# ChenDavidTimothy/mujoco-template

Hardware: AMD Instinct MI355X
Metric: env-steps/sec (whole node), humanoid batch=4096 random-ctrl rollout (higher is better)
Workload: dtype f32

## Files before the change

mujoco_template_amd/csrc/mjb_device.hpp:

```cpp
#pragma once
#include "mjb_types.hpp"

#ifdef MJB_HOST_EMU
#include <cmath>
#include "mjb_hostemu.hpp"
#define MJB_DEV static inline
#define MJB_DEVM inline
#define MJB_DEV_CALL static __attribute__((noinline))
#else
#include <hip/hip_runtime.h>
#define MJB_DEV __device__ __forceinline__
#define MJB_DEVM __device__ __forceinline__
#define MJB_DEV_CALL __device__ __attribute__((noinline))
#endif

#ifdef MJB_HOST_EMU
#define MJB_MFMA(a, b, acc) emu_mfma((a), (b), (acc))
#define MJB_BALLOT(p) emu_ballot(p)
#define MJB_RSQF(x) (1.0f / sqrtf(x))
#define MJB_RCPF(x) (1.0f / (x))
#define MJB_MEMTIME() 0ull
#define MJB_OPAQUE1(a) ((void)0)
#define MJB_OPAQUE2(a, b) ((void)0)
#define MJB_OPAQUE9(a, b, c, d, e, f, g, h, i) ((void)0)
// ... 1418 lines not shown
        if (t_abs(det) >= (sizeof(T) == 4 ? (T)1e-6 * ma * mc : Num<T>::minval())) {
          x1 = (mc * u - mb * v) / det; x2 = (ma * v - mb * u) / det;
          if (x1 > s1[1]) { x1 = s1[1]; x2 = (v - mb * s1[1]) / mc; }
          else if (x1 < -s1[1]) { x1 = -s1[1]; x2 = (v + mb * s1[1]) / mc; }
          if (x2 > s2[1]) { x2 = s2[1]; x1 = t_min(t_max((u - mb * s2[1]) / ma, -s1[1]), s1[1]); }
          else if (x2 < -s2[1]) { x2 = -s2[1]; x1 = t_min(t_max((u + mb * s2[1]) / ma, -s1[1]), s1[1]); }
          T v1[3] = {p1[0] + z1[0] * x1, p1[1] + z1[1] * x1, p1[2] + z1[2] * x1};
          T v2[3] = {p2[0] + z2[0] * x2, p2[1] + z2[1] * x2, p2[2] + z2[2] * x2};
          n = nc_sphere_sphere(v1, s1[0], v2, s2[0], margin, rc[0]);
        } else {
#pragma unroll
          for (int k = 0; k < 4; k++) {
            if (n >= 2) continue;
            bool ok;
            if (k < 2) { x1 = k == 0 ? s1[1] : -s1[1]; x2 = (v - mb * x1) / mc; ok = x2 >= -s2[1] && x2 <= s2[1]; }
            else { x2 = k == 2 ? s2[1] : -s2[1]; x1 = (u - mb * x2) / ma; ok = x1 >= -s1[1] && x1 <= s1[1]; }
            if (!ok) continue;
            T v1[3] = {p1[0] + z1[0] * x1, p1[1] + z1[1] * x1, p1[2] + z1[2] * x1};
            T v2[3] = {p2[0] + z2[0] * x2, p2[1] + z2[1] * x2, p2[2] + z2[2] * x2};
            RawCon<T> tmp;
            if (nc_sphere_sphere(v1, s1[0], v2, s2[0], margin, tmp)) { if (n == 0) rc[0] = tmp; else rc[1] = tmp; n++; }
          }
        }
      }
    }
    int total, off = gscan_small<G>(n, lane, total);
#pragma unroll
    for (int k = 0; k < 4; k++) {
      if (k < n) {
        int slot = ncon + off + k;
        if (slot < m.ncon_max) {
          const RawCon<T>& r = rc[k];
          T f[9] = {r.n[0], r.n[1], r.n[2], r.yh[0], r.yh[1], r.yh[2], 0, 0, 0};
          normalize3(f);
          if (dot3(f + 3, f + 3) < (T)0.25) {
            f[3] = f[4] = f[5] = 0;
            if (f[1] < (T)0.5 && f[1] > (T)-0.5) f[4] = 1; else f[5] = 1;
          }
          T d = dot3(f, f + 3);
          f[3] -= d * f[0]; f[4] -= d * f[1]; f[5] -= d * f[2];
          normalize3(f + 3);
          T* o = con + slot * CON_STRIDE;
          o[0] = r.dist; o[1] = r.pos[0]; o[2] = r.pos[1]; o[3] = r.pos[2];
#pragma unroll
          for (int a = 0; a < 6; a++) o[4 + a] = f[a];
          o[10] = prm_row<PRM_PAIR_FRICTION>(c, m.pair_friction, 5 * m.npair)[5 * p];
          con_pair[slot] = p;
        }
      }
    }
    int newn = ncon + total;
    if (newn > m.ncon_max) { dropped += newn - (ncon > m.ncon_max ? ncon : m.ncon_max); }
    ncon = newn;
  }
}

template <typename T, int G> MJB_DEV void collision(Ctx<T>& c) {
  MJB_ENV(c); T* w = c.w; const int lane = c.lane;
  T *gx = w + L.geom_xpos, *gm = w + L.geom_xmat;
  int ncon = 0, dropped = 0;
  if (m.nefc_max * m.nv < G) {
    for (int base = 0; base < m.npair; base += G) collide_pass<T, G>(c, base + lane, base + lane < m.npair, ncon, dropped);
  } else {
    int* cand = (int*)(w + L.efc_J);
    int nl = 0;
    for (int base = 0; base < m.npair; base += G) {
      const int p = base + lane;
      bool keep = false;
      if (p < m.npair) {
        const int g1 = m.pair_geom1[p], g2 = m.pair_geom2[p];
        const T cull = m.pair_cull[p];
        T d[3] = {gx[3 * g2] - gx[3 * g1], gx[3 * g2 + 1] - gx[3 * g1 + 1], gx[3 * g2 + 2] - gx[3 * g1 + 2]};
        if (cull < 0) {
          T nz[3] = {gm[9 * g1 + 2], gm[9 * g1 + 5], gm[9 * g1 + 8]};
          keep = dot3(d, nz) <= -cull * (T)1.00001 + (T)1e-6;
        } else {
          T r = cull * (T)1.00001 + (T)1e-6;
          keep = dot3(d, d) <= r * r;
        }
      }
      int total, off = gscan_small<G>(keep ? 1 : 0, lane, total);
      if (nl + total > G) {
        gsync<G>();
        collide_pass<T, G>(c, lane < nl ? cand[lane] : 0, lane < nl, ncon, dropped);
        gsync<G>();
        nl = 0;
      }
      if (keep) cand[nl + off] = p;
      nl += total;
    }
    gsync<G>();
    if (nl > 0) collide_pass<T, G>(c, lane < nl ? cand[lane] : 0, lane < nl, ncon, dropped);
  }
  c.con_dropped += dropped;
  c.ncon = ncon < m.ncon_max ? ncon : m.ncon_max;
  gsync<G>();
}

template <typename T> MJB_DEV void row_imp_R(T pos, T margin, const T* solimp, T diagApprox, T& imp, T& R) {
  T dmin = t_min(t_max(solimp[0], MJB_MINIMP), MJB_MAXIMP), dmax = t_min(t_max(solimp[1], MJB_MINIMP), MJB_MAXIMP);
  T width = t_max(solimp[2], (T)0), mid = t_min(t_max(solimp[3], MJB_MINIMP), MJB_MAXIMP), power = t_max(solimp[4], (T)1);
  if (dmin == dmax || width <= Num<T>::minval()) imp = (T)0.5 * (dmin + dmax);
  else {
    T x = t_abs(pos - margin) / width;
    if (x >= 1) imp = dmax;
    else if (x <= 0) imp = dmin;
    else {
      T y;
      if (power == 1) y = x;
#ifdef MJB_SPEC_SOLIMP_POWER_1_OR_2
      else y = x <= mid ? x * x / mid : 1 - (1 - x) * (1 - x) / (1 - mid);
#else
      else if (power == 2) y = x <= mid ? x * x / mid : 1 - (1 - x) * (1 - x) / (1 - mid);
      else if (x <= mid) y = t_pow(x, power) / t_pow(mid, power - 1);
      else y = 1 - t_pow(1 - x, power) / t_pow(1 - mid, power - 1);
#endif
      imp = dmin + y * (dmax - dmin);
    }
  }
  R = t_max(Num<T>::minval(), (1 - imp) * diagApprox / imp);
}
template <typename T> MJB_DEV void row_params(ModelRef<T> m, T pos, T margin, const T* solref, const T* solimp, T diagApprox, T& K, T& B, T& imp, T& R) {
  T dmin = t_min(t_max(solimp[0], MJB_MINIMP), MJB_MAXIMP), dmax = t_min(t_max(solimp[1], MJB_MINIMP), MJB_MAXIMP);
  T width = t_max(solimp[2], (T)0), mid = t_min(t_max(solimp[3], MJB_MINIMP), MJB_MAXIMP), power = t_max(solimp[4], (T)1);
  if (dmin == dmax || width <= Num<T>::minval()) imp = (T)0.5 * (dmin + dmax);
  else {
    T x = t_abs(pos - margin) / width;
    if (x >= 1) imp = dmax;
    else if (x <= 0) imp = dmin;
    else {
      T y;
      if (power == 1) y = x;
#ifdef MJB_SPEC_SOLIMP_POWER_1_OR_2
      else y = x <= mid ? x * x / mid : 1 - (1 - x) * (1 - x) / (1 - mid);
#else
      else if (power == 2) y = x <= mid ? x * x / mid : 1 - (1 - x) * (1 - x) / (1 - mid);
      else if (x <= mid) y = t_pow(x, power) / t_pow(mid, power - 1);
      else y = 1 - t_pow(1 - x, power) / t_pow(1 - mid, power - 1);
#endif
      imp = dmin + y * (dmax - dmin);
    }
  }
  if (solref[0] > 0) {
    T tc = t_max(solref[0], 2 * m.timestep), dr = solref[1];
    K = 1 / t_max(Num<T>::minval(), dmax * dmax * tc * tc * dr * dr);
    B = 2 / t_max(Num<T>::minval(), dmax * tc);
  } else {
    K = -solref[0] / t_max(Num<T>::minval(), dmax * dmax);
    B = -solref[1] / t_max(Num<T>::minval(), dmax);
  }
  R = t_max(Num<T>::minval(), (1 - imp) * diagApprox / imp);
}

template <typename T, int G> MJB_DEV void make_constraint(Ctx<T>& c) {
  MJB_ENV(c); T* w = c.w; const int lane = c.lane, nv = m.nv, cap = m.nefc_max;
  T *qpos = w + L.qpos, *qvel = w + L.qvel, *J = w + L.efc_J, *epos = w + L.efc_pos, *eD = w + L.efc_D, *earef = w + L.efc_aref;
  T *eK = w + L.efc_jar, *eB = w + L.efc_jv, *eI = w + L.efc_force;
  T *emargin = w + L.efc_KBI;
  int *etype = c.wi + L.i_efc_type, *con_pair = c.wi + L.i_con_pair;
  T *con = w + L.con, *tl = w + L.ten_length, *tj = w + L.ten_J;
  int nefc = 0, dropped = 0;
  {
    const int nobj = m.njnt + m.ntendon;
    for (int base = 0; base < nobj; base += G) {
      const int k = base + lane;
      const bool isj = k < m.njnt;
      const int o = isj ? k : k - m.njnt;
      int cnt = 0;
      T dist[2] = {0, 0}, margin = 0;
      bool act[2] = {false, false};
      T rec[12];
      if (k < nobj && m.lim_i[2 * k]) {
        const int vi = m.lim_i[2 * k + 1];
#pragma unroll
        for (int q = 0; q < 11; q++) rec[q] = m.lim_f[12 * k + q];
        T value = isj ? qpos[vi] : tl[vi];
        margin = rec[2];
        dist[0] = value - rec[0]; dist[1] = rec[1] - value;
        act[0] = dist[0] < margin; act[1] = dist[1] < margin;
        cnt = (int)act[0] + (int)act[1];
      }
      int total, off = gscan_small<G>(cnt, lane, total);
      int row = nefc + off;
      if (cnt > 0) {
#pragma unroll
        for (int sd = 0; sd < 2; sd++) {
          if (act[sd]) {
            if (row < cap) {
              T imp, R;
              row_imp_R(dist[sd], margin, rec + 6, rec[3], imp, R);
              etype[row] = (isj ? EFC_LIMIT_JOINT : EFC_LIMIT_TENDON) | ((o * 2 + sd) << 9);
              epos[row] = dist[sd]; emargin[row] = margin; eD[row] = 1 / R; eK[row] = rec[4]; eB[row] = rec[5]; eI[row] = imp;
            }
            row++;
          }
        }
      }
      int newn = nefc + total;
      if (newn > cap) dropped += newn - (nefc > cap ? nefc : cap);
      nefc = newn;
    }
  }
  if (nefc > cap) nefc = cap;
  int nlimit = nefc;
  for (int base = 0; base < c.ncon; base += G) {
    int ci = base + lane, rows = 0, p = 0;
    T dist = 0, mu = 0, incm = 0;
    if (ci < c.ncon) {
      p = con_pair[ci] & 0xffff;
      dist = con[ci * CON_STRIDE]; mu = con[ci * CON_STRIDE + 10];
      incm = m.pair_kb[4 * p];
      if (dist < incm) rows = m.pair_condim[p] == 1 ? 1 : 4;
    }
    int total, off = gscan_small<G>(rows, lane, total);
    int row = nefc + off;
    if (ci < c.ncon) {
      bool fits = rows > 0 && row + rows <= cap;
      con_pair[ci] = p | ((fits ? row + 1 : 0) << 16);
      if (fits) {
        const T tran = m.pair_kb[4 * p + 1], K = m.pair_kb[4 * p + 2], B = m.pair_kb[4 * p + 3];
        T si[5] = {m.pair_solimp[5 * p], m.pair_solimp[5 * p + 1], m.pair_solimp[5 * p + 2], m.pair_solimp[5 * p + 3], m.pair_solimp[5 * p + 4]};
        T imp, R;
        if (rows == 1) row_imp_R(dist, incm, si, tran, imp, R);
        else {
          row_imp_R(dist, incm, si, tran + mu * mu * tran, imp, R);
          R = t_max(Num<T>::minval(), 2 * mu * mu * R);
        }
        for (int r = 0; r < rows; r++) {
          etype[row + r] = (rows == 1 ? EFC_CONTACT_FRICTIONLESS : EFC_CONTACT_PYRAMIDAL) | (ci << 9);
          epos[row + r] = dist; emargin[row + r] = incm; eD[row + r] = 1 / R; eK[row + r] = K; eB[row + r] = B; eI[row + r] = imp;
        }
      }
    }
    int newn = nefc + total;
    if (newn > cap) dropped += newn - (nefc > cap ? nefc : cap);
    nefc = newn;
  }
  if (nefc > cap) {
    int last = nlimit;
    for (int ci = lane; ci < c.ncon; ci += G) {
      int a = (con_pair[ci] >> 16) - 1;
      if (a >= 0) { int p = con_pair[ci] & 0xffff; int e = a + (m.pair_condim[p] == 1 ? 1 : 4); if (e > last) last = e; }
    }
    nefc = gmaxi<G>(last);
  }
  c.nefc = nefc; c.efc_dropped += dropped;
  gsync<G>();
  {
    int tot = nlimit << m.nvshift;
    for (int idx = lane; idx < tot; idx += G) {
      int r = idx >> m.nvshift, i = idx & (m.nvp - 1);
      if (i >= nv) continue;
      int id_ = etype[r] >> 9, o = id_ >> 1, s = id_ & 1;
      T sign = s == 0 ? (T)1 : (T)-1, v;
      if ((etype[r] & 0xff) == EFC_LIMIT_JOINT) v = (i == m.jnt_dofadr[o]) ? sign : (T)0;
      else v = sign * tj[o * nv + i];
      J[r * nv + i] = v;
    }
  }
  {
    int tot = c.ncon << m.nvshift;
    for (int idx = lane; idx < tot; idx += G) {
      int ci = idx >> m.nvshift, i = idx & (m.nvp - 1);
      if (i >= nv) continue;
      int row = (con_pair[ci] >> 16) - 1;
      if (row < 0) continue;
      int p = con_pair[ci] & 0xffff;
      int b1 = m.pair_body[2 * p], b2 = m.pair_body[2 * p + 1];
      const T* cc = con + ci * CON_STRIDE;
      T pos[3] = {cc[1], cc[2], cc[3]}, j1[3], j2[3], dj[3];
      jac_col<T>(c, b1, i, pos, j1, (T*)0);
      jac_col<T>(c, b2, i, pos, j2, (T*)0);
      dj[0] = j2[0] - j1[0]; dj[1] = j2[1] - j1[1]; dj[2] = j2[2] - j1[2];
      T jn = cc[4] * dj[0] + cc[5] * dj[1] + cc[6] * dj[2];
      if (m.pair_condim[p] == 1) J[row * nv + i] = jn;
      else {
        T mu = cc[10], nrm[3] = {cc[4], cc[5], cc[6]}, t1[3] = {cc[7], cc[8], cc[9]}, t2[3];
        cross3(t2, nrm, t1);
        T jt1 = mu * dot3(t1, dj), jt2 = mu * dot3(t2, dj);
        J[row * nv + i] = jn + jt1; J[(row + 1) * nv + i] = jn - jt1;
        J[(row + 2) * nv + i] = jn + jt2; J[(row + 3) * nv + i] = jn - jt2;
      }
    }
  }
  gsync<G>();
  const VecLds<T> xv{qvel};
  for (int r = lane; r < nefc; r += G) {
    T v = dot_lds(J + r * nv, 1, xv, nv);
    earef[r] = -eB[r] * v - eK[r] * eI[r] * (epos[r] - emargin[r]);
  }
  gsync<G>();
}

template <typename T, int G> MJB_DEV void vel_bias_passive(Ctx<T>& c) {
  MJB_ENV(c); T* w = c.w; const int lane = c.lane, nv = m.nv;
  T *cvel = w + L.cvel, *cacc = w + L.cacc, *cfrc = w + L.cfrc, *cdof = w + L.cdof, *cdd = w + L.cdof_dot, *cin = w + L.cinert;
  T *qvel = w + L.qvel, *qpos = w + L.qpos;
  if (lane == 0) {
#pragma unroll
    for (int k = 0; k < 6; k++) { cvel[k] = 0; cfrc[k] = 0; }
    const T MJB_CONST* gravity = prm_row<PRM_GRAVITY>(c, m.gravity, 3);
    cacc[0] = cacc[1] = cacc[2] = 0; cacc[3] = -gravity[0]; cacc[4] = -gravity[1]; cacc[5] = -gravity[2];
  }
  gsync<G>();
  for (int b = 1 + lane; b < m.nbody; b += G) {
    int da = m.body_dofadr[b], dn = m.body_dofnum[b];
    T dv[6] = {0, 0, 0, 0, 0, 0};
    for (int j = da; j < da + dn; j++) {
      T qv = qvel[j];
#pragma unroll
      for (int q = 0; q < 6; q++) dv[q] += cdof[6 * j + q] * qv;
    }
#pragma unroll
    for (int q = 0; q < 6; q++) cvel[6 * b + q] = dv[q];
  }
  gsync<G>();
  tree_forward_sum<T, G, 6>(c, cvel);
  for (int j = lane; j < nv; j += G) {
    const int p = m.dof_irec[6 * j + 1], first = m.dof_irec[6 * j + 2], gs = m.dof_irec[6 * j + 3];
    T tmp[6] = {0, 0, 0, 0, 0, 0};
    if (gs >= 0) {
      T cv[6], cd[6];
#pragma unroll
      for (int q = 0; q < 6; q++) { cv[q] = cvel[6 * p + q]; cd[q] = cdof[6 * j + q]; }
      for (int k = first; k < gs; k++) {
        T qv = qvel[k];
#pragma unroll
        for (int q = 0; q < 6; q++) cv[q] += cdof[6 * k + q] * qv;
      }
      cross_motion(tmp, cv, cd);
    }
#pragma unroll
    for (int q = 0; q < 6; q++) cdd[6 * j + q] = tmp[q];
  }
  gsync<G>();
  for (int b = 1 + lane; b < m.nbody; b += G) {
    int da = m.body_dofadr[b], dn = m.body_dofnum[b];
    T da6[6] = {0, 0, 0, 0, 0, 0};
    for (int j = da; j < da + dn; j++) {
      T qv = qvel[j];
#pragma unroll
      for (int q = 0; q < 6; q++) da6[q] += cdd[6 * j + q] * qv;
    }
    if (m.body_depth[b] == 1) {
#pragma unroll
      for (int q = 0; q < 6; q++) da6[q] += cacc[q];
    }
#pragma unroll
    for (int q = 0; q < 6; q++) cacc[6 * b + q] = da6[q];
  }
  gsync<G>();
  tree_forward_sum<T, G, 6>(c, cacc);
  for (int b = 1 + lane; b < m.nbody; b += G) {
    T in[10], cv[6], ca[6], f[6], t1[6], t2[6];
#pragma unroll
    for (int k = 0; k < 10; k++) in[k] = cin[10 * b + k];
#pragma unroll
    for (int k = 0; k < 6; k++) { cv[k] = cvel[6 * b + k]; ca[k] = cacc[6 * b + k]; }
    mul_inert_vec(f, in, ca);
    mul_inert_vec(t1, in, cv);
    cross_force(t2, cv, t1);
#pragma unroll
    for (int k = 0; k < 6; k++) cfrc[6 * b + k] = f[k] + t2[k];
  }
  gsync<G>();
  tree_backward_sum<T, G, 6>(c, cfrc, m.nround_inner, 1);
  T* bfrc = w + L.bfrc;
  if (m.has_fluid) {
    T *xipos = w + L.xipos, *ximat = w + L.ximat, *sc = w + L.subtree_com;
    for (int b = lane; b < m.nbody; b += G) {
      T mass = prm_row<PRM_BODY_MASS>(c, m.body_mass, m.nbody)[b];
#pragma unroll
      for (int k = 0; k < 6; k++) bfrc[6 * b + k] = 0;
      if (b == 0 || mass < Num<T>::minval()) continue;
      const T MJB_CONST* inertia = prm_row<PRM_BODY_INERTIA>(c, m.body_inertia, 3 * m.nbody);
      T I0 = inertia[3 * b], I1 = inertia[3 * b + 1], I2 = inertia[3 * b + 2];
      T box[3] = {t_sqrt(t_max(Num<T>::minval(), I1 + I2 - I0) / mass * 6), t_sqrt(t_max(Num<T>::minval(), I0 + I2 - I1) / mass * 6), t_sqrt(t_max(Num<T>::minval(), I0 + I1 - I2) / mass * 6)};
      int r = m.body_rootid[b];
      T cv[6], off[3], lin[3], t[3], im[9], lvel[6], lfrc[6] = {0, 0, 0, 0, 0, 0};
#pragma unroll
      for (int k = 0; k < 6; k++) cv[k] = cvel[6 * b + k];
#pragma unroll
      for (int k = 0; k < 3; k++) off[k] = xipos[3 * b + k] - sc[3 * r + k];
#pragma unroll
      for (int k = 0; k < 9; k++) im[k] = ximat[9 * b + k];
      cross3(t, cv, off);
      lin[0] = cv[3] + t[0]; lin[1] = cv[4] + t[1]; lin[2] = cv[5] + t[2];
      mulmatTvec3(lvel, im, cv);
      mulmatTvec3(lvel + 3, im, lin);
      if (m.viscosity > 0) {
        T diam = (box[0] + box[1] + box[2]) / 3;
#pragma unroll
        for (int k = 0; k < 3; k++) { lfrc[k] = -MJB_PI * diam * diam * diam * m.viscosity * lvel[k]; lfrc[3 + k] = -3 * MJB_PI * diam * m.viscosity * lvel[3 + k]; }
      }
      if (m.density > 0) {
        lfrc[3] -= (T)0.5 * m.density * box[1] * box[2] * t_abs(lvel[3]) * lvel[3];
        lfrc[4] -= (T)0.5 * m.density * box[0] * box[2] * t_abs(lvel[4]) * lvel[4];
        lfrc[5] -= (T)0.5 * m.density * box[0] * box[1] * t_abs(lvel[5]) * lvel[5];
        T b0 = box[0] * box[0], b1 = box[1] * box[1], b2 = box[2] * box[2];
        lfrc[0] -= m.density * box[0] * (b1 * b1 + b2 * b2) * t_abs(lvel[0]) * lvel[0] / 64;
        lfrc[1] -= m.density * box[1] * (b0 * b0 + b2 * b2) * t_abs(lvel[1]) * lvel[1] / 64;
        lfrc[2] -= m.density * box[2] * (b0 * b0 + b1 * b1) * t_abs(lvel[2]) * lvel[2] / 64;
      }
      T o1[3], o2[3];
      mulmatvec3(o1, im, lfrc);
      mulmatvec3(o2, im, lfrc + 3);
#pragma unroll
      for (int k = 0; k < 3; k++) { bfrc[6 * b + k] = o1[k]; bfrc[6 * b + 3 + k] = o2[k]; }
    }
    gsync<G>();
  }
  T *qb = w + L.qfrc_bias, *qp = w + L.qfrc_passive;
  for (int i = lane; i < nv; i += G) {
    const int b = m.dof_irec[6 * i], qa = m.dof_irec[6 * i + 4];
    T v = 0;
#pragma unroll
    for (int k = 0; k < 6; k++) v += cdof[6 * i + k] * cfrc[6 * b + k];
    qb[i] = v;
    T pf = -prm_get<PRM_DOF_DAMPING>(c, m.dof_frec, nv, i, 4 * i) * qvel[i];
    if (qa >= 0) pf -= m.dof_frec[4 * i + 1] * (qpos[qa] - m.dof_frec[4 * i + 2]);
    if (m.has_fluid) {
      T* xipos = w + L.xipos;
      for (int bb = 1; bb < m.nbody; bb++) {
        if (!((m.body_dofmask[bb] >> i) & 1ull)) continue;
        T pt[3] = {xipos[3 * bb], xipos[3 * bb + 1], xipos[3 * bb + 2]}, jp[3], jr[3];
        jac_col<T>(c, bb, i, pt, jp, jr);
        pf += jp[0] * bfrc[6 * bb + 3] + jp[1] * bfrc[6 * bb + 4] + jp[2] * bfrc[6 * bb + 5] + jr[0] * bfrc[6 * bb] + jr[1] * bfrc[6 * bb + 1] + jr[2] * bfrc[6 * bb + 2];
      }
    }
    qp[i] = pf;
  }
  gsync<G>();
}

template <typename T, int G> MJB_DEV void actuation_forces(Ctx<T>& c) {
  MJB_ENV(c); T* w = c.w; const int lane = c.lane, nv = m.nv;
  T *ctrl = w + L.ctrl, *af = w + L.act_force, *qpos = w + L.qpos, *qvel = w + L.qvel;
  for (int a = lane; a < m.nu; a += G) {
    int grp = m.actuator_group[a];
    T force = 0;
    if (!(grp >= 0 && grp < 31 && ((MJB_OPT(c, disableactuator) >> grp) & 1))) {
      T u = ctrl[a];
      if (m.actuator_ctrllimited[a]) u = t_min(t_max(u, m.actuator_ctrlrange[2 * a]), m.actuator_ctrlrange[2 * a + 1]);
      force = prm_row<PRM_ACT_GAINPRM>(c, m.actuator_gainprm, 3 * m.nu)[3 * a] * u;
      if (m.actuator_biastype[a] == 1) {
        T len = 0, vel = 0;
        if (m.actuator_trntype[a] == TRN_JOINT) {
          int j = m.actuator_trnid[2 * a];
          const T MJB_CONST* gear = prm_row<PRM_ACT_GEAR>(c, m.actuator_gear, 6 * m.nu);
          len = gear[6 * a] * qpos[m.jnt_qposadr[j]];
          vel = gear[6 * a] * qvel[m.jnt_dofadr[j]];
        }
        const T MJB_CONST* bias = prm_row<PRM_ACT_BIASPRM>(c, m.actuator_biasprm, 3 * m.nu);
        force += bias[3 * a] + bias[3 * a + 1] * len + bias[3 * a + 2] * vel;
      }
      if (m.actuator_forcelimited[a]) force = t_min(t_max(force, m.actuator_forcerange[2 * a]), m.actuator_forcerange[2 * a + 1]);
    }
    af[a] = force;
  }
  gsync<G>();
  T *qa = w + L.qfrc_actuator, *qs = w + L.qfrc_smooth, *qas = w + L.qacc_smooth, *qb = w + L.qfrc_bias, *qp = w + L.qfrc_passive;
  T *sx = w + L.site_xpos, *sm = w + L.site_xmat;
  for (int i = lane; i < nv; i += G) {
    T s = 0;
    const T MJB_CONST* gear = prm_row<PRM_ACT_GEAR>(c, m.actuator_gear, 6 * m.nu);
    for (int k = m.dofact_adr[i]; k < m.dofact_adr[i + 1]; k++) { int a = m.dofact_act[k]; s += gear[6 * a] * af[a]; }
    for (int k = 0; k < m.nsiteact; k++) {
      int a = m.siteact[k], id = m.actuator_trnid[2 * a], b = m.site_bodyid[id];
      if (!((m.body_dofmask[b] >> i) & 1ull)) continue;
      T g[6], R[9], f[3], tq[3], pt[3] = {sx[3 * id], sx[3 * id + 1], sx[3 * id + 2]}, jp[3], jr[3];
#pragma unroll
      for (int q = 0; q < 6; q++) g[q] = gear[6 * a + q];
#pragma unroll
      for (int q = 0; q < 9; q++) R[q] = sm[9 * id + q];
      mulmatvec3(f, R, g);
      mulmatvec3(tq, R, g + 3);
      jac_col<T>(c, b, i, pt, jp, jr);
      s += (dot3(jp, f) + dot3(jr, tq)) * af[a];
    }
    qa[i] = s;
    T fs = qp[i] - qb[i] + s;
    qs[i] = fs; qas[i] = fs;
  }
  gsync<G>();
}
template <typename T, int G> MJB_DEV void actuation_acceleration(Ctx<T>& c) {
  actuation_forces<T, G>(c);
  factor_W<T, G>(c, 0, c.w + c.lp->qacc_smooth);
}

template <typename T, int G> MJB_DEV bool jt_split(int nv) { return G == 64 && nv <= 32; }
template <typename T, int G> MJB_DEV T jt_dot(const T* J, const T* f, int nefc, int nv, int lane) {
  const int h = lane >> 5, i = lane & 31, n2 = (nefc + 1) >> 1;
  const int r0 = h ? n2 : 0, cnt = h ? nefc - n2 : n2;
  T p = i < nv ? dot_lds(J + r0 * nv + i, nv, VecLds<T>{f + r0}, cnt) : (T)0;
  return half_sum(p);
}

template <typename T, int G> MJB_DEV T solver_cost(Ctx<T>& c, const T* qacc, bool store) {
  MJB_ENV(c); T* w = c.w; const int lane = c.lane, nv = m.nv, nefc = c.nefc;
  T *M = w + L.M, *J = w + L.efc_J, *Ma = w + L.Ma, *jar = w + L.efc_jar, *aref = w + L.efc_aref, *D = w + L.efc_D, *force = w + L.efc_force;
  T *qs = w + L.qfrc_smooth, *qas = w + L.qacc_smooth;
  T part = 0;
  const VecLds<T> xq{qacc};
  for (int rho = lane; rho < nv + nefc; rho += G) {
    const bool ism = rho < nv;
    const int r = ism ? rho : rho - nv;
    T s = dot_lds(ism ? M + r * nv : J + r * nv, 1, xq, nv);
    if (ism) {
      Ma[r] = s;
      part += (T)0.5 * (s - qs[r]) * (qacc[r] - qas[r]);
    } else {
      s -= aref[r];
      jar[r] = s;
      if (s < 0) { part += (T)0.5 * D[r] * s * s; if (store) force[r] = -D[r] * s; }
      else if (store) force[r] = 0;
    }
  }
  T cost = gsum<T, G>(part);
  gsync<G>();
  return cost;
}

template <typename T> MJB_DEV bool mark_active_row(int* etype, T* dw, int r, T sj, T d) {
  const int act = sj < 0 ? 1 : 0, t = etype[r];
  etype[r] = (t & ~0x100) | (act << 8);
  dw[r] = act ? d : (T)0;
  return ((t >> 8) & 1) != act;
}
template <typename T, int G> MJB_DEV T newton_direction(Ctx<T>& c, bool rebuild, T gtol2) {
  MJB_ENV(c); T* w = c.w; const int lane = c.lane, nv = m.nv, nefc = c.nefc;
  T *M = w + L.M, *W = w + L.W, *J = w + L.efc_J, *Ma = w + L.Ma, *force = w + L.efc_force;
  T *grad = w + L.grad, *search = w + L.search, *qs = w + L.qfrc_smooth;
  T gpart = 0;
  for (int rp_ = MJB_REP_N(c, REP_GRAD); rp_ > 0; rp_--) {
  gpart = 0;
  if (jt_split<T, G>(nv)) {
    const int i = lane & 31;
    T jf = jt_dot<T, G>(J, force, nefc, nv, lane);
    if (lane < nv) { T g = Ma[i] - qs[i] - jf; grad[i] = g; search[i] = -g; gpart = g * g; }
  } else {
    for (int i = lane; i < nv; i += G) {
      T g = Ma[i] - qs[i] - dot_lds(J + i, nv, VecLds<T>{force}, nefc);
      grad[i] = g; search[i] = -g;
      gpart += g * g;
    }
  }
  }
  T gn = gsum<T, G>(gpart);
  gsync<G>();
  if (gn < gtol2) return gn;
  MJB_COUNT(c, PH_CNT_DIR); if (rebuild) MJB_COUNT(c, PH_CNT_FACT);
  for (int rp_ = MJB_REP_N(c, rebuild ? REP_CHOL : REP_REUSE); rp_ > 1; rp_--) {
    if (rebuild) factor_W<T, G>(c, 1, search);
    else if (fused_inverse_path<T, G>(nv)) { gsync<G>(); if constexpr (sizeof(T) == 4) mfma_solve32(W, w + L.tmp, search, nv, lane); }
    for (int i = lane; i < nv; i += G) search[i] = -grad[i];
    gsync<G>();
  }
  if (rebuild) factor_W<T, G>(c, 1, search);
  else if (fused_inverse_path<T, G>(nv)) { gsync<G>(); if constexpr (sizeof(T) == 4) mfma_solve32(W, w + L.tmp, search, nv, lane); }
  else chol_solve<T, G>(W, w + L.tmp, search, nv, lane);
  return gn;
}

template <typename T, int G> MJB_DEV void solve_constraints(Ctx<T>& c) {
  MJB_ENV(c); T* w = c.w; const int lane = c.lane, nv = m.nv, nefc = c.nefc;
  T *qacc = w + L.qacc, *ws = w + L.qacc_ws, *qas = w + L.qacc_smooth, *qc = w + L.qfrc_constraint;
  c.niter = 0;
  if (nefc == 0) {
    for (int i = lane; i < nv; i += G) { T a = qas[i]; qacc[i] = a; ws[i] = a; qc[i] = 0; }
    gsync<G>();
    return;
  }
  T *M = w + L.M, *J = w + L.efc_J, *Ma = w + L.Ma, *jar = w + L.efc_jar, *jv = w + L.efc_jv, *D = w + L.efc_D, *force = w + L.efc_force;
  T *search = w + L.search, *Mv = w + L.Mv, *qs = w + L.qfrc_smooth;
  int* etype = c.wi + L.i_efc_type;
  T cost;
  for (int rp_ = MJB_REP_N(c, REP_WARM); rp_ > 0; rp_--) {
    T *aref = w + L.efc_aref;
    T pa = 0, pb = 0;
    const VecLds<T> xa{qas}, xb{ws};
    for (int rho = lane; rho < nv + nefc; rho += G) {
      const bool ism = rho < nv;
      const int r = ism ? rho : rho - nv;
      const T* row = ism ? M + r * nv : J + r * nv;
      T sa = dot_lds(row, 1, xa, nv), sb = dot_lds(row, 1, xb, nv);
      if (ism) {
        Ma[r] = sa; Mv[r] = sb;
        pa += (T)0.5 * (sa - qs[r]) * (qas[r] - qas[r]);
        pb += (T)0.5 * (sb - qs[r]) * (ws[r] - qas[r]);
      } else {
        sa -= aref[r]; sb -= aref[r];
        jar[r] = sa; jv[r] = sb;
        if (sa < 0) pa += (T)0.5 * D[r] * sa * sa;
        if (sb < 0) pb += (T)0.5 * D[r] * sb * sb;
      }
    }
    const T cost_a = gsum<T, G>(pa), cost_b = gsum<T, G>(pb);
    gsync<G>();
    const bool wsw = cost_b < cost_a;
    cost = wsw ? cost_b : cost_a;
    for (int i = lane; i < nv; i += G) { qacc[i] = wsw ? ws[i] : qas[i]; if (wsw) Ma[i] = Mv[i]; }
    for (int r = lane; r < nefc; r += G) {
      const T sj = wsw ? jv[r] : jar[r], d = D[r];
      if (wsw) jar[r] = sj;
      force[r] = sj < 0 ? -d * sj : (T)0;
      mark_active_row<T>(etype, jv, r, sj, d);
    }
    gsync<G>();
  }
  bool rebuild_wanted = true;
  const T scale = 1 / (m.meaninertia * (T)(nv > 1 ? nv : 1));
  const int max_iter = MJB_OPT(c, iterations);
  const T tolerance = MJB_OPT(c, tolerance), gtol = tolerance / scale, gtol2 = gtol * gtol;
  for (int iter = 0; iter < max_iter; iter++) {
    MJB_STAMP(c, PH_SOLVE);
    T gn = newton_direction<T, G>(c, rebuild_wanted, gtol2);
    MJB_STAMP(c, PH_SOL_DIR);
    if (gn < gtol2) break;
    T p1 = 0, p2 = 0;
    const VecLds<T> xs{search};
    for (int rp_ = MJB_REP_N(c, REP_MV); rp_ > 0; rp_--) {
    p1 = 0; p2 = 0;
    for (int rho = lane; rho < nv + nefc; rho += G) {
      const bool ism = rho < nv;
      const int r = ism ? rho : rho - nv;
      T sacc = dot_lds(ism ? M + r * nv : J + r * nv, 1, xs, nv);
      if (ism) { Mv[r] = sacc; p1 += search[r] * (Ma[r] - qs[r]); p2 += search[r] * sacc; }
      else jv[r] = sacc;
    }
    }
    T g1 = gsum<T, G>(p1), g2 = gsum<T, G>(p2);
    gsync<G>();
    MJB_STAMP(c, PH_SOL_MV);
    T alpha = 0;
    for (int rp_ = MJB_REP_N(c, REP_LS); rp_ > 0; rp_--) {
      alpha = 0;
      const bool inreg = nefc <= G;
      T x0r = 0, jwr = 0, djr = 0;
      if (inreg && lane < nefc) { x0r = jar[lane]; jwr = jv[lane]; djr = D[lane] * jwr; }
      T lo = 0, hi = -1;
      for (int it = 0; it < 50; it++) {
        T d1p = 0, d2p = 0;
        if (inreg) {
          T x = x0r + alpha * jwr;
          if (x < 0) { d1p = djr * x; d2p = djr * jwr; }
        } else {
          for (int r = lane; r < nefc; r += G) {
            T x = jar[r] + alpha * jv[r];
            if (x < 0) { T dj = D[r] * jv[r]; d1p += dj * x; d2p += dj * jv[r]; }
          }
        }
        T d1 = g1 + alpha * g2 + gsum<T, G>(d1p), d2 = g2 + gsum<T, G>(d2p);
        if (it == 0 && d1 >= 0) { alpha = 0; break; }
        if (d2 < Num<T>::minval()) break;
        if (t_abs(d1) < (sizeof(T) == 4 ? (T)1e-6 : (T)1e-14) * (t_abs(g1) + Num<T>::minval())) break;
        if (d1 < 0) lo = alpha; else hi = alpha;
        T an = alpha - d1 / d2;
        bool newton = true;
        if (an <= lo || (hi >= 0 && an >= hi)) { an = hi >= 0 ? (T)0.5 * (lo + hi) : 2 * alpha + (T)1e-3; newton = false; }
        if (an == alpha) break;
        bool flip = false;
        if (inreg) flip = ((x0r + alpha * jwr) < 0) != ((x0r + an * jwr) < 0);
        else for (int r = lane; r < nefc; r += G) flip |= ((jar[r] + alpha * jv[r]) < 0) != ((jar[r] + an * jv[r]) < 0);
        const bool anyflip = gany<G>(flip);
        alpha = an;
        MJB_COUNT(c, PH_CNT_LS);
        if (newton && !anyflip) break;
      }
    }
    MJB_STAMP(c, PH_SOL_LS);
    if (alpha == 0) break;
    T part = 0;
    for (int i = lane; i < nv; i += G) {
      T a = qacc[i] + alpha * search[i], ma = Ma[i] + alpha * Mv[i];
      qacc[i] = a; Ma[i] = ma;
      part += (T)0.5 * (ma - qs[i]) * (a - qas[i]);
    }
    bool chg = false;
    for (int r = lane; r < nefc; r += G) {
      const T sj = jar[r] + alpha * jv[r], d = D[r];
      jar[r] = sj;
      if (sj < 0) { part += (T)0.5 * d * sj * sj; force[r] = -d * sj; } else force[r] = 0;
      chg = mark_active_row<T>(etype, jv, r, sj, d) || chg;
    }
    T old = cost;
    cost = gsum<T, G>(part);
    rebuild_wanted = gany<G>(chg);
    gsync<G>();
    c.niter = iter + 1;
    if (scale * (old - cost) < tolerance) break;
  }
  if (jt_split<T, G>(nv)) {
    T jf = jt_dot<T, G>(J, force, nefc, nv, lane);
    if (lane < nv) { qc[lane] = jf; ws[lane] = qacc[lane]; }
  } else {
    for (int i = lane; i < nv; i += G) { qc[i] = dot_lds(J + i, nv, VecLds<T>{force}, nefc); ws[i] = qacc[i]; }
  }
  gsync<G>();
}

template <typename T, typename TS, int G> MJB_DEV void sensors(const Ctx<T>& c, TS* dst) {
  ModelRef<T> m = MJB_MODEL_OF(c.mp); LayRef L = *c.lp; const T* w = c.w; const int lane = c.lane;
  for (int s = lane; s < m.nsensor; s += G) {
    TS* out = dst + m.sensor_adr[s];
    int id = m.sensor_objid[s], st = m.sensor_type[s];
    if (st == SENS_JOINTPOS) { out[0] = (TS)w[L.qpos + m.jnt_qposadr[id]]; continue; }
    int b = m.site_bodyid[id];
    T R[9];
#pragma unroll
    for (int k = 0; k < 9; k++) R[k] = w[L.site_xmat + 9 * id + k];
    if (st == SENS_GYRO) {
      T wv[3] = {w[L.cvel + 6 * b], w[L.cvel + 6 * b + 1], w[L.cvel + 6 * b + 2]}, o3[3];
      mulmatTvec3(o3, R, wv);
      out[0] = (TS)o3[0]; out[1] = (TS)o3[1]; out[2] = (TS)o3[2];
    } else if (st == SENS_FRAMEQUAT) {
      T bq[4] = {w[L.xquat + 4 * b], w[L.xquat + 4 * b + 1], w[L.xquat + 4 * b + 2], w[L.xquat + 4 * b + 3]};
      T sq[4] = {m.site_quat[4 * id], m.site_quat[4 * id + 1], m.site_quat[4 * id + 2], m.site_quat[4 * id + 3]}, q[4];
      quat_mul(q, bq, sq);
      quat_normalize(q);
      out[0] = (TS)q[0]; out[1] = (TS)q[1]; out[2] = (TS)q[2]; out[3] = (TS)q[3];
    } else if (st == SENS_ACCEL) {
      T cv[6], ca[6];
#pragma unroll
      for (int k = 0; k < 6; k++) { cv[k] = w[L.cvel + 6 * b + k]; ca[k] = w[L.cacc + 6 * b + k]; }
      for (int i = 0; i < m.nv; i++) {
        if (!((m.body_dofmask[b] >> i) & 1ull)) continue;
        T qa = w[L.qacc + i];
#pragma unroll
        for (int k = 0; k < 6; k++) ca[k] += w[L.cdof + 6 * i + k] * qa;
      }
      int r = m.body_rootid[b];
      T dif[3] = {w[L.site_xpos + 3 * id] - w[L.subtree_com + 3 * r], w[L.site_xpos + 3 * id + 1] - w[L.subtree_com + 3 * r + 1], w[L.site_xpos + 3 * id + 2] - w[L.subtree_com + 3 * r + 2]};
      T t[3], vlin[3], alin[3], wl[3], vl[3], al[3], cr[3];
      cross3(t, cv, dif); vlin[0] = cv[3] + t[0]; vlin[1] = cv[4] + t[1]; vlin[2] = cv[5] + t[2];
      cross3(t, ca, dif); alin[0] = ca[3] + t[0]; alin[1] = ca[4] + t[1]; alin[2] = ca[5] + t[2];
      mulmatTvec3(wl, R, cv); mulmatTvec3(vl, R, vlin); mulmatTvec3(al, R, alin);
      cross3(cr, wl, vl);
      out[0] = (TS)(al[0] + cr[0]); out[1] = (TS)(al[1] + cr[1]); out[2] = (TS)(al[2] + cr[2]);
    } else { out[0] = 0; }
  }
}

template <typename T, int G> MJB_DEV void forward_position(Ctx<T>& c) {
  MJB_STAMP(c, PH_OTHER);
  MJB_PHASE_CALL(c, PH_KIN, (kinematics<T, G>(c))); MJB_STAMP(c, PH_KIN);
  MJB_PHASE_CALL(c, PH_COM, (com_pos<T, G>(c))); MJB_STAMP(c, PH_COM);
  MJB_PHASE_CALL(c, PH_COLL, (collision<T, G>(c))); MJB_STAMP(c, PH_COLL);
  MJB_PHASE_CALL(c, PH_CRB, (crb_factor<T, G>(c))); MJB_STAMP(c, PH_CRB);
}
template <typename T, int G> MJB_DEV void forward_velocity(Ctx<T>& c) {
  MJB_PHASE_CALL(c, PH_CONS, (make_constraint<T, G>(c))); MJB_STAMP(c, PH_CONS);
  MJB_PHASE_CALL(c, PH_VEL, (vel_bias_passive<T, G>(c))); MJB_STAMP(c, PH_VEL);
}
template <typename T, int G> MJB_DEV void forward_acceleration(Ctx<T>& c) {
  MJB_PHASE_CALL(c, PH_ACT, (actuation_acceleration<T, G>(c))); MJB_STAMP(c, PH_ACT);
  solve_constraints<T, G>(c); MJB_STAMP(c, PH_SOLVE);
  if (c.mp->nsensor > 0) { sensors<T, T, G>(c, c.w + c.lp->sens); gsync<G>(); }
}
template <typename T, int G> MJB_DEV void forward(Ctx<T>& c) {
  forward_position<T, G>(c);
  forward_velocity<T, G>(c);
  if (c.skip_dynamics) return;
  forward_acceleration<T, G>(c);
}

template <typename T, int G> MJB_DEV void integrate_pos(ModelRef<T> m, T* qpos, const T* qvel, T h, int lane) {
  for (int j = lane; j < m.njnt; j += G) {
    int qa = m.jnt_irec[6 * j + 1], da = m.jnt_irec[6 * j + 2];
    if (m.jnt_irec[6 * j] == JNT_FREE) {
      qpos[qa] += h * qvel[da]; qpos[qa + 1] += h * qvel[da + 1]; qpos[qa + 2] += h * qvel[da + 2];
      T q[4] = {qpos[qa + 3], qpos[qa + 4], qpos[qa + 5], qpos[qa + 6]}, wv[3] = {qvel[da + 3], qvel[da + 4], qvel[da + 5]};
      quat_integrate(q, wv, h);
      qpos[qa + 3] = q[0]; qpos[qa + 4] = q[1]; qpos[qa + 5] = q[2]; qpos[qa + 6] = q[3];
    } else qpos[qa] += h * qvel[da];
  }
}

template <typename T, int G> MJB_DEV void euler(Ctx<T>& c, const mjb_f16v* inv = nullptr) {
  MJB_ENV(c); T* w = c.w; const int lane = c.lane, nv = m.nv;
  T *qacc = w + L.qacc, *qvel = w + L.qvel, *qpos = w + L.qpos, *tmpv = w + L.Mv, *M = w + L.M, *W = w + L.W;
  T h = m.timestep;
  if (has_damping(c, m.has_damping)) {
    T *qs = w + L.qfrc_smooth, *qc = w + L.qfrc_constraint;
    if (MJB_REPEATS(c, PH_INTEG)) {
      for (int i = lane; i < nv; i += G) tmpv[i] = qs[i] + qc[i];
      gsync<G>();
      factor_W<T, G>(c, 2, tmpv);
      gsync<G>();
    }
    for (int i = lane; i < nv; i += G) tmpv[i] = qs[i] + qc[i];
    gsync<G>();
#ifndef MJB_HOST_EMU
    if constexpr (sizeof(T) == 4 && G == 64) {
      if (inv) mfma_sweep_apply32(*inv, w + L.tmp, nv, lane, tmpv);
      else factor_W<T, G>(c, 2, tmpv);
    } else
#endif
    factor_W<T, G>(c, 2, tmpv);
  } else {
    for (int i = lane; i < nv; i += G) tmpv[i] = qacc[i];
    gsync<G>();
  }
  for (int i = lane; i < nv; i += G) qvel[i] += h * tmpv[i];
  gsync<G>();
  integrate_pos<T, G>(m, qpos, qvel, h, lane);
  gsync<G>();
}

template <typename T, int G> MJB_DEV void rk4_stage(Ctx<T>& c, int st) {
  MJB_ENV(c); T* w = c.w; const int lane = c.lane, nv = m.nv, nq = m.nq;
  T *qacc = w + L.qacc, *qvel = w + L.qvel, *qpos = w + L.qpos;
  T *X0q = w + L.rk, *X0v = X0q + nq, *Fv = X0v + nv, *Fa = Fv + 4 * nv, *dv = Fa + 4 * nv;
  const T h = m.timestep;
  if (st == 0) {
    for (int i = lane; i < nq; i += G) X0q[i] = qpos[i];
    for (int i = lane; i < nv; i += G) X0v[i] = qvel[i];
  }
  for (int i = lane; i < nv; i += G) { Fv[st * nv + i] = qvel[i]; Fa[st * nv + i] = qacc[i]; }
  gsync<G>();
  for (int i = lane; i < nv; i += G) {
    T sv, sa;
    if (st < 3) { T a = st == 2 ? (T)1 : (T)0.5; sv = a * Fv[st * nv + i]; sa = a * Fa[st * nv + i]; }
    else {
      sv = (Fv[i] + 2 * Fv[nv + i] + 2 * Fv[2 * nv + i] + Fv[3 * nv + i]) * (T)(1.0 / 6);
      sa = (Fa[i] + 2 * Fa[nv + i] + 2 * Fa[2 * nv + i] + Fa[3 * nv + i]) * (T)(1.0 / 6);
    }
    dv[i] = sv; qvel[i] = X0v[i] + h * sa;
  }
  for (int i = lane; i < nq; i += G) qpos[i] = X0q[i];
  gsync<G>();
  integrate_pos<T, G>(m, qpos, dv, h, lane);
  gsync<G>();
}

MJB_DEV unsigned philox_first(unsigned c0, unsigned c1, unsigned c2, unsigned c3, unsigned k0, unsigned k1) {
  for (int r = 0; r < 10; r++) {
    unsigned long long p0 = 0xD2511F53ull * c0, p1 = 0xCD9E8D57ull * c2;
    unsigned n0 = (unsigned)(p1 >> 32) ^ c1 ^ k0, n1 = (unsigned)p1, n2 = (unsigned)(p0 >> 32) ^ c3 ^ k1, n3 = (unsigned)p0;
    c0 = n0; c1 = n1; c2 = n2; c3 = n3;
    k0 += 0x9E3779B9u; k1 += 0xBB67AE85u;
  }
  return c0;
}
template <typename T, int G> MJB_DEV void random_ctrl(ModelRef<T> m, T* ctrl, unsigned seed, unsigned env, unsigned step, T scale, int lane) {
  for (int a = lane; a < m.nu; a += G) {
    unsigned r = philox_first(env, step, (unsigned)a, 0u, seed, 0x5EEDu);
    T u = (T)(r >> 8) * (T)(1.0 / 16777216.0);
    T lo = -1, hi = 1;
    if (m.actuator_ctrllimited[a]) { lo = m.actuator_ctrlrange[2 * a]; hi = m.actuator_ctrlrange[2 * a + 1]; }
    ctrl[a] = (T)0.5 * (lo + hi) + (T)0.5 * (hi - lo) * scale * (2 * u - 1);
  }
}

template <typename T, int G> MJB_DEV void feedback_ctrl(Ctx<T>& c, ArgsRef a, unsigned env, unsigned step) {
  MJB_ENV(c); T* w = c.w; const int lane = c.lane, nv = m.nv, nu = m.nu;
  auto K = (const T MJB_CONST*)a.fb_K; auto u0 = (const T MJB_CONST*)a.fb_u0;
  auto q0 = (const T MJB_CONST*)a.fb_q0; auto v0 = (const T MJB_CONST*)a.fb_v0;
  T *dx = w + L.grad, *qpos = w + L.qpos, *qvel = w + L.qvel, *ctrl = w + L.ctrl;
  for (int j = lane; j < m.njnt; j += G) {
    int qa = m.jnt_qposadr[j], da = m.jnt_dofadr[j];
    if (m.jnt_type[j] == JNT_FREE) {
      dx[da] = qpos[qa] - q0[qa]; dx[da + 1] = qpos[qa + 1] - q0[qa + 1]; dx[da + 2] = qpos[qa + 2] - q0[qa + 2];
      T qa4[4] = {q0[qa + 3], q0[qa + 4], q0[qa + 5], q0[qa + 6]}, qb4[4] = {qpos[qa + 3], qpos[qa + 4], qpos[qa + 5], qpos[qa + 6]}, r[3];
      quat_sub(r, qa4, qb4);
      dx[da + 3] = r[0]; dx[da + 4] = r[1]; dx[da + 5] = r[2];
    } else dx[da] = qpos[qa] - q0[qa];
  }
  for (int i = lane; i < nv; i += G) dx[nv + i] = qvel[i] - v0[i];
  gsync<G>();
  for (int act = lane; act < nu; act += G) {
    T u = u0[act];
    for (int k = 0; k < 2 * nv; k++) u -= K[act * 2 * nv + k] * dx[k];
    if (a.fb_nsteps > 0) {
      const long idx = ((long)step + (long)env * a.fb_env_stride) % a.fb_nsteps;
      u += ((const T MJB_CONST*)a.fb_noise_std)[act] * ((const T MJB_CONST*)a.fb_noise_tab)[idx * nu + act];
    }
    if (m.actuator_ctrllimited[act]) u = t_min(t_max(u, m.actuator_ctrlrange[2 * act]), m.actuator_ctrlrange[2 * act + 1]);
    ctrl[act] = u;
  }
  gsync<G>();
}

template <typename T, typename TS, int G> MJB_DEV_CALL void sequence_ctrl(T* ctrl, ArgsRef a, int nu, int env, int step, int lane) {
  const TS* src = (const TS*)a.ctrl_seq + (long)step * a.ctrl_step_stride + (long)env * a.ctrl_env_stride;
  for (int i = lane; i < nu; i += G) ctrl[i] = (T)src[i];
}

template <typename T, typename TS, int G> MJB_DEV void inverse_dynamics(Ctx<T>& c, TS* inv_out, TS* moment_out) {
  MJB_ENV(c); T* w = c.w; const int lane = c.lane, nv = m.nv, nefc = c.nefc;
  T *J = w + L.efc_J, *aref = w + L.efc_aref, *D = w + L.efc_D, *force = w + L.efc_force, *qacc = w + L.qacc, *M = w + L.M;
  T *qb = w + L.qfrc_bias, *qp = w + L.qfrc_passive, *qc = w + L.qfrc_constraint;
  for (int r = lane; r < nefc; r += G) {
    T jar = dot_lds(J + r * nv, 1, VecLds<T>{qacc}, nv) - aref[r];
    force[r] = jar < 0 ? -D[r] * jar : (T)0;
  }
  gsync<G>();
  for (int i = lane; i < nv; i += G) {
    T fc = dot_lds(J + i, nv, VecLds<T>{force}, nefc);
    T ma = dot_lds(M + i * nv, 1, VecLds<T>{qacc}, nv);
    qc[i] = fc;
    inv_out[i] = (TS)(ma + qb[i] - qp[i] - fc);
  }
  T *sx = w + L.site_xpos, *sm = w + L.site_xmat;
  for (int idx = lane; idx < m.nu * nv; idx += G) {
    int a = idx / nv, i = idx - a * nv, id = m.actuator_trnid[2 * a];
    T v = 0;
    const T MJB_CONST* gear = prm_row<PRM_ACT_GEAR>(c, m.actuator_gear, 6 * m.nu);
    if (m.actuator_trntype[a] == TRN_JOINT) v = (i == m.jnt_dofadr[id]) ? gear[6 * a] : (T)0;
    else {
      int b = m.site_bodyid[id];
      if ((m.body_dofmask[b] >> i) & 1ull) {
        T g[6], R[9], f[3], tq[3], pt[3] = {sx[3 * id], sx[3 * id + 1], sx[3 * id + 2]}, jp[3], jr[3];
#pragma unroll
        for (int q = 0; q < 6; q++) g[q] = gear[6 * a + q];
// ... 470 lines not shown
```

Baseline: 54.04 million.

## Prefetch limit records before CRB and fold final constraint force into last iteration

Limit-constraint model records (lim_i/lim_f) for the first lane batch are now loaded into registers right after collision, before crb_factor, so their global-memory latency overlaps CRB work rather than stalling make_constraint. Separately, the post-solver qfrc_constraint J^T·force product is now computed only at loop exit. The gradient pass also stores J^T·force into qfrc_constraint as a side effect. The prefetch holds about 13 extra live registers across crb_factor, which could raise register pressure and lower occupancy.

```diff
diff --git a/mujoco_template_amd/csrc/mjb_device.hpp b/mujoco_template_amd/csrc/mjb_device.hpp
--- a/mujoco_template_amd/csrc/mjb_device.hpp
+++ b/mujoco_template_amd/csrc/mjb_device.hpp
@@ -1594,7 +1594,22 @@
   R = t_max(Num<T>::minval(), (1 - imp) * diagApprox / imp);
 }
 
-template <typename T, int G> MJB_DEV void make_constraint(Ctx<T>& c) {
+template <typename T> struct ConsRec { int on, vi; T f[11]; };
+template <typename T, int G> MJB_DEV ConsRec<T> cons_fetch(const Ctx<T>& c) {
+  MJB_ENV(c); const int nobj = m.njnt + m.ntendon;
+  ConsRec<T> r;
+  r.on = 0; r.vi = 0;
+#pragma unroll
+  for (int q = 0; q < 11; q++) r.f[q] = 0;
+  if (nobj > 0) {
+    const int k = c.lane < nobj ? c.lane : nobj - 1;
+    r.on = m.lim_i[2 * k]; r.vi = m.lim_i[2 * k + 1];
+#pragma unroll
+    for (int q = 0; q < 11; q++) r.f[q] = m.lim_f[12 * k + q];
+  }
+  return r;
+}
+template <typename T, int G> MJB_DEV void make_constraint(Ctx<T>& c, const ConsRec<T>& first) {
   MJB_ENV(c); T* w = c.w; const int lane = c.lane, nv = m.nv, cap = m.nefc_max;
   T *qpos = w + L.qpos, *qvel = w + L.qvel, *J = w + L.efc_J, *epos = w + L.efc_pos, *eD = w + L.efc_D, *earef = w + L.efc_aref;
   T *eK = w + L.efc_jar, *eB = w + L.efc_jv, *eI = w + L.efc_force;
@@ -1612,10 +1627,10 @@
       T dist[2] = {0, 0}, margin = 0;
       bool act[2] = {false, false};
       T rec[12];
-      if (k < nobj && m.lim_i[2 * k]) {
-        const int vi = m.lim_i[2 * k + 1];
-#pragma unroll
-        for (int q = 0; q < 11; q++) rec[q] = m.lim_f[12 * k + q];
+      if (k < nobj && (base == 0 ? first.on : m.lim_i[2 * k])) {
+        const int vi = base == 0 ? first.vi : m.lim_i[2 * k + 1];
+#pragma unroll
+        for (int q = 0; q < 11; q++) rec[q] = base == 0 ? first.f[q] : m.lim_f[12 * k + q];
         T value = isj ? qpos[vi] : tl[vi];
         margin = rec[2];
         dist[0] = value - rec[0]; dist[1] = rec[1] - value;
@@ -1734,6 +1749,8 @@
   gsync<G>();
 }
 
+template <typename T, int G> MJB_DEV void make_constraint(Ctx<T>& c) { make_constraint<T, G>(c, cons_fetch<T, G>(c)); }
+
 template <typename T, int G> MJB_DEV void vel_bias_passive(Ctx<T>& c) {
   MJB_ENV(c); T* w = c.w; const int lane = c.lane, nv = m.nv;
   T *cvel = w + L.cvel, *cacc = w + L.cacc, *cfrc = w + L.cfrc, *cdof = w + L.cdof, *cdd = w + L.cdof_dot, *cin = w + L.cinert;
@@ -1973,18 +1990,19 @@
 template <typename T, int G> MJB_DEV T newton_direction(Ctx<T>& c, bool rebuild, T gtol2) {
   MJB_ENV(c); T* w = c.w; const int lane = c.lane, nv = m.nv, nefc = c.nefc;
   T *M = w + L.M, *W = w + L.W, *J = w + L.efc_J, *Ma = w + L.Ma, *force = w + L.efc_force;
-  T *grad = w + L.grad, *search = w + L.search, *qs = w + L.qfrc_smooth;
+  T *grad = w + L.grad, *search = w + L.search, *qs = w + L.qfrc_smooth, *qc = w + L.qfrc_constraint;
   T gpart = 0;
   for (int rp_ = MJB_REP_N(c, REP_GRAD); rp_ > 0; rp_--) {
   gpart = 0;
   if (jt_split<T, G>(nv)) {
     const int i = lane & 31;
     T jf = jt_dot<T, G>(J, force, nefc, nv, lane);
-    if (lane < nv) { T g = Ma[i] - qs[i] - jf; grad[i] = g; search[i] = -g; gpart = g * g; }
+    if (lane < nv) { T g = Ma[i] - qs[i] - jf; grad[i] = g; search[i] = -g; qc[i] = jf; gpart = g * g; }
   } else {
     for (int i = lane; i < nv; i += G) {
-      T g = Ma[i] - qs[i] - dot_lds(J + i, nv, VecLds<T>{force}, nefc);
-      grad[i] = g; search[i] = -g;
+      T jf = dot_lds(J + i, nv, VecLds<T>{force}, nefc);
+      T g = Ma[i] - qs[i] - jf;
+      grad[i] = g; search[i] = -g; qc[i] = jf;
       gpart += g * g;
     }
   }
@@ -2003,6 +2021,17 @@
   else if (fused_inverse_path<T, G>(nv)) { gsync<G>(); if constexpr (sizeof(T) == 4) mfma_solve32(W, w + L.tmp, search, nv, lane); }
   else chol_solve<T, G>(W, w + L.tmp, search, nv, lane);
   return gn;
+}
+
+template <typename T, int G> MJB_DEV void constraint_force(Ctx<T>& c) {
+  MJB_ENV(c); T* w = c.w; const int lane = c.lane, nv = m.nv, nefc = c.nefc;
+  T *J = w + L.efc_J, *force = w + L.efc_force, *qc = w + L.qfrc_constraint;
+  if (jt_split<T, G>(nv)) {
+    T jf = jt_dot<T, G>(J, force, nefc, nv, lane);
+    if (lane < nv) qc[lane] = jf;
+  } else {
+    for (int i = lane; i < nv; i += G) qc[i] = dot_lds(J + i, nv, VecLds<T>{force}, nefc);
+  }
 }
 
 template <typename T, int G> MJB_DEV void solve_constraints(Ctx<T>& c) {
@@ -2131,14 +2160,10 @@
     rebuild_wanted = gany<G>(chg);
     gsync<G>();
     c.niter = iter + 1;
-    if (scale * (old - cost) < tolerance) break;
-  }
-  if (jt_split<T, G>(nv)) {
-    T jf = jt_dot<T, G>(J, force, nefc, nv, lane);
-    if (lane < nv) { qc[lane] = jf; ws[lane] = qacc[lane]; }
-  } else {
-    for (int i = lane; i < nv; i += G) { qc[i] = dot_lds(J + i, nv, VecLds<T>{force}, nefc); ws[i] = qacc[i]; }
-  }
+    if (scale * (old - cost) < tolerance || iter + 1 >= max_iter) { constraint_force<T, G>(c); break; }
+  }
+  if (max_iter <= 0) constraint_force<T, G>(c);
+  for (int i = lane; i < nv; i += G) ws[i] = qacc[i];
   gsync<G>();
 }
 
@@ -2184,15 +2209,18 @@
   }
 }
 
-template <typename T, int G> MJB_DEV void forward_position(Ctx<T>& c) {
+template <typename T, int G> MJB_DEV void forward_position(Ctx<T>& c, ConsRec<T>* cons = nullptr) {
   MJB_STAMP(c, PH_OTHER);
   MJB_PHASE_CALL(c, PH_KIN, (kinematics<T, G>(c))); MJB_STAMP(c, PH_KIN);
   MJB_PHASE_CALL(c, PH_COM, (com_pos<T, G>(c))); MJB_STAMP(c, PH_COM);
   MJB_PHASE_CALL(c, PH_COLL, (collision<T, G>(c))); MJB_STAMP(c, PH_COLL);
+  if (cons) *cons = cons_fetch<T, G>(c);
   MJB_PHASE_CALL(c, PH_CRB, (crb_factor<T, G>(c))); MJB_STAMP(c, PH_CRB);
 }
-template <typename T, int G> MJB_DEV void forward_velocity(Ctx<T>& c) {
-  MJB_PHASE_CALL(c, PH_CONS, (make_constraint<T, G>(c))); MJB_STAMP(c, PH_CONS);
+template <typename T, int G> MJB_DEV void forward_velocity(Ctx<T>& c, const ConsRec<T>* cons = nullptr) {
+  if (cons) { MJB_PHASE_CALL(c, PH_CONS, (make_constraint<T, G>(c, *cons))); }
+  else { MJB_PHASE_CALL(c, PH_CONS, (make_constraint<T, G>(c))); }
+  MJB_STAMP(c, PH_CONS);
   MJB_PHASE_CALL(c, PH_VEL, (vel_bias_passive<T, G>(c))); MJB_STAMP(c, PH_VEL);
 }
 template <typename T, int G> MJB_DEV void forward_acceleration(Ctx<T>& c) {
@@ -2201,8 +2229,9 @@
   if (c.mp->nsensor > 0) { sensors<T, T, G>(c, c.w + c.lp->sens); gsync<G>(); }
 }
 template <typename T, int G> MJB_DEV void forward(Ctx<T>& c) {
-  forward_position<T, G>(c);
-  forward_velocity<T, G>(c);
+  ConsRec<T> cons;
+  forward_position<T, G>(c, &cons);
+  forward_velocity<T, G>(c, &cons);
   if (c.skip_dynamics) return;
   forward_acceleration<T, G>(c);
 }
```

After: 54.28 million, median of 6. Within noise of the previous version (+0.4%).
